# slimgroup/dfno

Hardware: NVIDIA H100
Metric: 3D Navier-Stokes FNO training step (fwd+loss+bwd+Adam) samples/sec, whole job, device-timed, max over ranks (higher is better)
Workload: dtype bf16; 1 GPU; model=FNO3d+t 128^3x20t width 20 modes (12, 12, 12, 10) blocks 4, global_batch=1, seq_len=41943040, parallelism=y-pencil 1x1 (model parallel: field over y, spectral weights over kz), step=forward + DistributedRelativeLpLoss + backward + Adam

## Files before the change

### dfno_b200/csrc/head_sm90.cu

```cuda
#include <type_traits>

#include "head_common.cuh"
#include "kernels.h"
#include "tma_host.h"

namespace dfno {
namespace {

constexpr int kStagesHF = 6;
constexpr int kGroupsHF = 2;
static_assert(kStagesHF % kGroupsHF == 0, "every ring stage must belong to one consumer warpgroup");
constexpr int kThreadsHF = 128 * kGroupsHF + 32;

struct HeadFwdParams {
  int B, C, KR;
  long long S, tiles_per_b;
  const float* w4b4;
  float* out;
  RowMap map;
};


template <int KR, bool kPad>
__device__ __forceinline__ void head_fwd_body(const CUtensorMap& tmH, const CUtensorMap& tmW3, const HeadFwdParams p,
                                              const PadRowMap pm) {
  extern __shared__ __align__(1024) uint8_t smem[];
  constexpr uint32_t w3_bytes = KR > 64 ? 32768u : 16384u;
  uint8_t* s_w3 = smem;
  uint8_t* s_a = smem + w3_bytes;
  constexpr uint32_t half_bytes = KR * 128;
  constexpr uint32_t stage_bytes = 2 * half_bytes;
  uint64_t* bars = reinterpret_cast<uint64_t*>(s_a + kStagesHF * stage_bytes);
  uint64_t* full = bars;
  uint64_t* empty = bars + 6;
  uint64_t* wfull = bars + 12;
  uint32_t* s_w4 = reinterpret_cast<uint32_t*>(bars + 14);
  float* s_b4 = reinterpret_cast<float*>(s_w4 + 64);

  const int warp = __shfl_sync(0xffffffffu, static_cast<int>(threadIdx.x >> 5), 0), lane = threadIdx.x & 31;
  const long long num_tiles = p.tiles_per_b * p.B;

  for (uint32_t i = threadIdx.x; i < kStagesHF * stage_bytes / 16; i += blockDim.x)
    reinterpret_cast<uint4*>(s_a)[i] = make_uint4(0, 0, 0, 0);
  __syncthreads();
  for (uint32_t i = threadIdx.x; i < kStagesHF * 2 * 16; i += blockDim.x) {
    const uint32_t hb = i >> 4, ch = i & 15;
    reinterpret_cast<uint2*>(s_a + hb * half_bytes + p.C * 128)[ch] = make_uint2(0x3F803F80u, 0x3F803F80u);
  }
  for (int i = threadIdx.x; i < 64; i += blockDim.x)
    s_w4[i] = h2_bits(h2_from_f32(p.w4b4[2 * i], p.w4b4[2 * i + 1]));
  if (threadIdx.x == 0) s_b4[0] = p.w4b4[kHidH];
  if (threadIdx.x == 0) {
    tma_prefetch_desc(&tmH); tma_prefetch_desc(&tmW3);
    for (int s = 0; s < kStagesHF; ++s) { mbar_init(&full[s], 1); mbar_init(&empty[s], 1); }
    mbar_init(wfull, 1);
    fence_barrier_init();
  }
  fence_proxy_async_smem();
  __syncthreads();

  if (warp == 4 * kGroupsHF) {
    if (lane == 0) {
      mbar_arrive_expect_tx(wfull, w3_bytes);
      tma_load_2d(s_w3, &tmW3, wfull, 0, 0);
      if constexpr (KR > 64) tma_load_2d(s_w3 + 16384, &tmW3, wfull, 64, 0);
      uint32_t s = 0, ph = 0;
      for (long long tile = blockIdx.x; tile < num_tiles; tile += gridDim.x) {
        const int b = static_cast<int>(tile / p.tiles_per_b);
        const int p0 = static_cast<int>((tile % p.tiles_per_b) * 128);
        mbar_wait(&empty[s], ph ^ 1);
        mbar_arrive_expect_tx(&full[s], 2u * p.C * 128);
        uint8_t* st = s_a + s * stage_bytes;
        tma_load_2d(st, &tmH, &full[s], p0, b * p.C);
        tma_load_2d(st + half_bytes, &tmH, &full[s], p0 + 64, b * p.C);
        if (++s == kStagesHF) { s = 0; ph ^= 1; }
      }
    }
    return;
  }
  const int q = warp & 3, g = warp >> 2, cq = lane & 3;
  const int my_row = frag_row(q, lane, cq);
  const float b4 = s_b4[0];
  const uint32_t w_addr = smem_u32(s_w3);
  uint32_t w4[16];
#pragma unroll
  for (int j = 0; j < 16; ++j) w4[j] = s_w4[4 * j + cq];
  mbar_wait(wfull, 0);
  float acc[128];
  long long n = 0;
  for (long long tile = blockIdx.x; tile < num_tiles; tile += gridDim.x, ++n) {
    if (n % kGroupsHF != g) continue;
    const uint32_t s = static_cast<uint32_t>(n % kStagesHF);
    const int b = static_cast<int>(tile / p.tiles_per_b);
    const long long pos = (tile % p.tiles_per_b) * 128 + my_row;
    mbar_wait(&full[s], (n / kStagesHF) & 1);
    const uint32_t abase = smem_u32(s_a + s * stage_bytes);
    wgmma_fence();
#pragma unroll
    for (int ks = 0; ks < KR / 16; ++ks) {
      const uint32_t w_k = KR > 64 ? (ks >> 2) * 16384 + (ks & 3) * 32 : ks * 32;
      wg_mma128<false, 1, 0>(acc, kHidH, gdesc_mn128(abase + ks * 2048, half_bytes, 1024), half_bytes,
                             gdesc_k128(w_addr + w_k), ks > 0 ? 1u : 0u);
    }
    wgmma_commit();
    wgmma_wait<0>();
    acc_fence(acc);
    if (q == 0 && lane == 0) mbar_arrive(&empty[s]);
    float out[4];
#pragma unroll
    for (int k = 0; k < 4; ++k) {
      const float* a = acc + 64 * (k >> 1) + 2 * (k & 1);
      float sum = 0.f;
#pragma unroll
      for (int half = 0; half < 2; ++half) {
        __half2 part = __float2half2_rn(0.f);
#pragma unroll
        for (int j = 8 * half; j < 8 * half + 8; ++j)
          part = __hfma2(gelu_h2(h2_from_f32(a[4 * j], a[4 * j + 1])), h2_of_bits(w4[j]), part);
        const float2 f = __half22float2(part);
        sum += f.x + f.y;
      }
      sum += __shfl_xor_sync(0xffffffffu, sum, 1);
      sum += __shfl_xor_sync(0xffffffffu, sum, 2);
      out[k] = sum;
    }
    if constexpr (kPad) {
      const long long o = pos < p.S ? pad_row_to_offset(pm, static_cast<uint32_t>(b * p.S + pos)) : -1;
      if (o >= 0) p.out[o] = b4 + pick4(out, cq);
    } else {
      if (pos < p.S) p.out[row_to_offset(p.map, static_cast<uint32_t>(b * p.S + pos))] = b4 + pick4(out, cq);
    }
  }
}

template <int KR>
__global__ void __launch_bounds__(kThreadsHF, 1)
head_fwd_kernel(const __grid_constant__ CUtensorMap tmH, const __grid_constant__ CUtensorMap tmW3,
                const HeadFwdParams p) {
  head_fwd_body<KR, false>(tmH, tmW3, p, PadRowMap{});
}

template <int KR>
__global__ void __launch_bounds__(kThreadsHF, 1)
head_fwd_pad_kernel(const __grid_constant__ CUtensorMap tmH, const __grid_constant__ CUtensorMap tmW3,
                    const HeadFwdParams p, const __grid_constant__ PadRowMap pm) {
  head_fwd_body<KR, true>(tmH, tmW3, p, pm);
}

constexpr int kMaxStagesHB = 6;
constexpr int kGroupsHB = 2;
constexpr int kThreadsHB = 128 * kGroupsHB + 128;
constexpr int kProducerRegsHB = 24, kConsumerRegsHB = 240;
static_assert(128 * kProducerRegsHB + 128 * kGroupsHB * kConsumerRegsHB <= 65536, "register file");
template <int KR>
constexpr bool kWideHB = KR > 48;
template <int KR>
constexpr bool kWsumSmem = KR > 32 && !kWideHB<KR>;
template <int KR>
constexpr int kWsumSmemW = !kWideHB<KR> ? 0 : KR > 64 ? 24 : 32;

struct HeadBwdParams {
  int B, C, KR, stages;
  long long S, tiles_per_b;
  const float* dout;
  const float* amax;
  const float* W4;
  float* gW3; float* gb3; float* gW4; float* gb4;
  RowMap map;
};

template <int KR, bool kPad>
__device__ __forceinline__ void head_bwd2_body(const CUtensorMap& tmH, const CUtensorMap& tmW3, const CUtensorMap& tmW3T,
                                               const CUtensorMap& tmG, const HeadBwdParams p, const PadRowMap pm) {
  extern __shared__ __align__(1024) uint8_t smem[];
  constexpr uint32_t half_bytes = KR * 128;
  constexpr uint32_t tile_bytes = 2 * half_bytes;
  constexpr uint32_t w3_bytes = KR > 64 ? 32768u : 16384u;
  uint8_t* s_w3 = smem;
  uint8_t* s_w3t = s_w3 + w3_bytes;
  uint8_t* s_p = s_w3t + tile_bytes;
  uint8_t* s_a = s_p + kGroupsHB * 32768;
  uint8_t* s_hs = s_a + p.stages * tile_bytes;
  uint8_t* s_g = kWideHB<KR> ? s_hs : s_hs + kGroupsHB * tile_bytes;
  float* s_wsum = reinterpret_cast<float*>(s_g + kGroupsHB * tile_bytes);
  uint64_t* bars = reinterpret_cast<uint64_t*>(s_wsum + (kWsumSmem<KR> ? 32 * 128 * kGroupsHB : 0) +
                                               kWsumSmemW<KR> * 128 * kGroupsHB);
  uint64_t* a_full = bars;
  uint64_t* a_empty = bars + 8;
  uint64_t* w_full = bars + 16;
  float* s_gb4 = reinterpret_cast<float*>(bars + 18);
  uint32_t* s_w4h = reinterpret_cast<uint32_t*>(bars + 20);
  float* s_gw4 = reinterpret_cast<float*>(s_w4h + 64);

  const int warp = __shfl_sync(0xffffffffu, static_cast<int>(threadIdx.x >> 5), 0), lane = threadIdx.x & 31;
  const long long num_tiles = p.tiles_per_b * p.B;

  for (uint32_t i = threadIdx.x; i < p.stages * tile_bytes / 16; i += blockDim.x)
    reinterpret_cast<uint4*>(s_a)[i] = make_uint4(0, 0, 0, 0);
  for (uint32_t i = threadIdx.x; i < kGroupsHB * tile_bytes / 16; i += blockDim.x)
    reinterpret_cast<uint4*>(s_hs)[i] = make_uint4(0, 0, 0, 0);
  __syncthreads();
  for (uint32_t i = threadIdx.x; i < static_cast<uint32_t>(p.stages) * 2 * 16; i += blockDim.x) {
    const uint32_t hb = i >> 4, ch = i & 15;
    reinterpret_cast<uint2*>(s_a + hb * half_bytes + p.C * 128)[ch] = make_uint2(0x3F803F80u, 0x3F803F80u);
  }
  if (threadIdx.x == 0) s_gb4[0] = 0.f;
  for (int i = threadIdx.x; i < 64; i += blockDim.x) s_w4h[i] = h2_bits(h2_from_f32(p.W4[2 * i], p.W4[2 * i + 1]));
  for (int i = threadIdx.x; i < kHidH; i += blockDim.x) s_gw4[i] = 0.f;
  if (threadIdx.x == 0) {
    tma_prefetch_desc(&tmH); tma_prefetch_desc(&tmW3); tma_prefetch_desc(&tmW3T); tma_prefetch_desc(&tmG);
    for (int s = 0; s < p.stages; ++s) { mbar_init(&a_full[s], 1); mbar_init(&a_empty[s], 1); }
    mbar_init(w_full, 1);
    fence_barrier_init();
  }
  fence_proxy_async_smem();
  __syncthreads();
  const float amax = *p.amax;
  const float scale = amax > 0.f ? exp2f(-ceilf(log2f(amax))) : 1.0f;

  if (warp >= 4 * kGroupsHB) {
    setmaxnreg_dec<kProducerRegsHB>();
    if (warp == 4 * kGroupsHB && lane == 0) {
      mbar_arrive_expect_tx(w_full, w3_bytes + tile_bytes);
      tma_load_2d(s_w3, &tmW3, w_full, 0, 0);
      if constexpr (KR > 64) tma_load_2d(s_w3 + 16384, &tmW3, w_full, 64, 0);
      tma_load_2d(s_w3t, &tmW3T, w_full, 0, 0);
      tma_load_2d(s_w3t + half_bytes, &tmW3T, w_full, 64, 0);
      uint32_t s = 0, ph = 0;
      for (long long tile = blockIdx.x; tile < num_tiles; tile += gridDim.x) {
        const int b = static_cast<int>(tile / p.tiles_per_b);
        const int p0 = static_cast<int>((tile % p.tiles_per_b) * 128);
        mbar_wait(&a_empty[s], ph ^ 1);
        mbar_arrive_expect_tx(&a_full[s], 2u * p.C * 128);
        uint8_t* st = s_a + s * tile_bytes;
        tma_load_2d(st, &tmH, &a_full[s], p0, b * p.C);
        tma_load_2d(st + half_bytes, &tmH, &a_full[s], p0 + 64, b * p.C);
        if (++s == static_cast<uint32_t>(p.stages)) { s = 0; ph ^= 1; }
      }
    }
    return;
  }

  setmaxnreg_inc<kConsumerRegsHB>();
  const int q = warp & 3, g = warp >> 2, cq = lane & 3;
  const int my_row = frag_row(q, lane, cq);
  const uint32_t barid = 1 + g;
  const bool leader = q == 0 && lane == 0;
  uint8_t* pbuf = s_p + g * 32768;
  uint8_t* hsbuf = s_hs + g * tile_bytes;
  uint8_t* gbuf = s_g + g * tile_bytes;
  const uint32_t w3_addr = smem_u32(s_w3), w3t_addr = smem_u32(s_w3t);
  const uint32_t p_addr = smem_u32(pbuf), hs_addr = smem_u32(hsbuf), g_addr = smem_u32(gbuf);
  const int mi = lane >> 3, mk = lane & 7;
  const uint32_t p_row = 16 * q + 8 * (mi & 1) + mk;
  const uint32_t g_chunk = 2 * q + (mi & 1);
  float acc_gb4 = 0.f;
  float wsum[32];
  float* my_wsum = s_wsum + (threadIdx.x & (128 * kGroupsHB - 1));
#pragma unroll
  for (int i = 0; i < 32; ++i) {
    if constexpr (kWsumSmem<KR>) my_wsum[i * 128 * kGroupsHB] = 0.f;
    else if constexpr (kWideHB<KR>) { if (i < kWsumSmemW<KR>) my_wsum[i * 128 * kGroupsHB] = 0.f; else wsum[i] = 0.f; }
    else wsum[i] = 0.f;
  }
  auto wsum_add = [&](int i, float d, float v) {
    if constexpr (kWsumSmem<KR>) my_wsum[i * 128 * kGroupsHB] = fmaf(d, v, my_wsum[i * 128 * kGroupsHB]);
    else if constexpr (kWideHB<KR>) {
      if (i < kWsumSmemW<KR>) my_wsum[i * 128 * kGroupsHB] = fmaf(d, v, my_wsum[i * 128 * kGroupsHB]);
      else wsum[i] = fmaf(d, v, wsum[i]);
    } else wsum[i] = fmaf(d, v, wsum[i]);
  };
  float d3[KR];
  uint32_t pa[2][4][4];
  auto mma2 = [&](float (&acc2)[KR], int kb) {
    if constexpr (!kWideHB<KR>) {
#pragma unroll
      for (int ks = 0; ks < 4; ++ks) {
        const uint64_t db = gdesc_k128(w3t_addr + kb * half_bytes + ks * 32);
        const uint32_t sc = (kb > 0 || ks > 0) ? 1u : 0u;
        wg_mma64_rs<KR, 0, 0>(acc2, pa[0][ks], db, sc);
        wg_mma64_rs<KR, 0, KR / 2>(acc2, pa[1][ks], db, sc);
      }
    }
  };
  auto mma2_group = [&](auto c0_, auto ng_, const float (&dk)[4]) {
    constexpr int c0 = decltype(c0_)::value, NG = decltype(ng_)::value;
    float a2[NG];
    wgmma_fence();
#pragma unroll
    for (int ks = 0; ks < 8; ++ks) {
      const uint32_t kb = ks >> 2, kk = ks & 3;
      wg_mma128<true, 0, 0>(a2, NG, gdesc_k128(p_addr + kb * 16384 + kk * 32), 8192,
                            gdesc_k128(w3t_addr + kb * half_bytes + c0 * 128 + kk * 32), ks > 0 ? 1u : 0u);
    }
    wgmma_commit();
    wgmma_wait<0>();
    acc_fence(a2);
#pragma unroll
    for (int mh = 0; mh < 2; ++mh) {
#pragma unroll
      for (int t = 0; t < NG / 16; ++t) {
        uint32_t r[4];
#pragma unroll
        for (int i = 0; i < 4; ++i) {
          const float* a = a2 + (NG / 2) * mh + 4 * (2 * t + (i >> 1)) + 2 * (i & 1);
          const float d = dk[2 * mh + (i & 1)];
          r[i] = pack_bf16x2(d * a[0], d * a[1]);
        }
        const uint32_t c = c0 + 16 * t + 8 * (mi >> 1) + mk;
        stmatrix_x4_trans(g_addr + mh * half_bytes + c * 128 + ((g_chunk ^ (c & 7)) << 4), r);
      }
    }
  };
  long long n = 0, mine = 0;
  mbar_wait(w_full, 0);
  for (long long tile = blockIdx.x; tile < num_tiles; tile += gridDim.x, ++n) {
    if (n % kGroupsHB != g) continue;
    const uint32_t s = static_cast<uint32_t>(n % p.stages);
    const int b = static_cast<int>(tile / p.tiles_per_b);
    const long long p0 = (tile % p.tiles_per_b) * 128;
    const long long pos = p0 + my_row;
    float dl;
    if constexpr (kPad) {
      const long long o = pos < p.S ? pad_row_to_offset(pm, static_cast<uint32_t>(b * p.S + pos)) : -1;
      dl = o >= 0 ? p.dout[o] : 0.f;
    } else {
      dl = pos < p.S ? p.dout[row_to_offset(p.map, static_cast<uint32_t>(b * p.S + pos))] : 0.f;
    }
    acc_gb4 += dl;
    float dk[4];
#pragma unroll
    for (int k = 0; k < 4; ++k) dk[k] = __shfl_sync(0xffffffffu, dl, (lane & ~3) | k);
    mbar_wait(&a_full[s], (n / p.stages) & 1);
    const uint32_t abase = smem_u32(s_a + s * tile_bytes);
    float acc2[KR];
    if constexpr (kWideHB<KR>) {
#pragma unroll
      for (int hq = 0; hq < 4; ++hq) {
        float acc[32];
        wgmma_fence();
#pragma unroll
        for (int ks = 0; ks < KR / 16; ++ks) {
          const uint32_t w_k = KR > 64 ? (ks >> 2) * 16384 + (ks & 3) * 32 : ks * 32;
          wg_mma128<false, 1, 0>(acc, 32, gdesc_mn128(abase + ks * 2048, half_bytes, 1024), half_bytes,
                                 gdesc_k128(w3_addr + hq * 4096 + w_k), ks > 0 ? 1u : 0u);
        }
        wgmma_commit();
        wgmma_wait<0>();
        acc_fence(acc);
        const int hh = hq >> 1;
#pragma unroll
        for (int mh = 0; mh < 2; ++mh) {
#pragma unroll
          for (int kq = 0; kq < 2; ++kq) {
            const int ks = 2 * (hq & 1) + kq;
            uint32_t pr[4];
            afrag_from_acc(acc + 16 * mh, kq, pr, [&](float lo, float hi, int i) {
              const int j = 2 * ks + (i >> 1);
              const GeluH2 vg = gelu_vg_h2(h2_from_f32(lo, hi));
              const float2 a = __half22float2(vg.value);
              const float d = dk[2 * mh + (i & 1)];
              wsum_add(16 * hh + 2 * j, d, a.x);
              wsum_add(16 * hh + 2 * j + 1, d, a.y);
              return h2_bits(__hmul2(vg.grad, h2_of_bits(s_w4h[32 * hh + 4 * j + cq])));
            });
            const uint32_t row = 64 * mh + p_row, chunk = 2 * ks + (mi >> 1);
            stmatrix_x4(p_addr + hh * 16384 + row * 128 + ((chunk ^ (row & 7)) << 4), pr);
          }
        }
      }
    } else {
#pragma unroll
      for (int hh = 0; hh < 2; ++hh) {
        float acc[64];
        wgmma_fence();
#pragma unroll
        for (int ks = 0; ks < KR / 16; ++ks)
          wg_mma128<false, 1, 0>(acc, 64, gdesc_mn128(abase + ks * 2048, half_bytes, 1024), half_bytes,
                                 gdesc_k128(w3_addr + hh * 8192 + ks * 32), ks > 0 ? 1u : 0u);
        wgmma_commit();
        wgmma_wait<0>();
        acc_fence(acc);
#pragma unroll
        for (int mh = 0; mh < 2; ++mh) {
#pragma unroll
          for (int ks = 0; ks < 4; ++ks) {
            afrag_from_acc(acc + 32 * mh, ks, pa[mh][ks], [&](float lo, float hi, int i) {
              const int j = 2 * ks + (i >> 1);
              const GeluH2 vg = gelu_vg_h2(h2_from_f32(lo, hi));
              const float2 a = __half22float2(vg.value);
              const float d = dk[2 * mh + (i & 1)];
              wsum_add(16 * hh + 2 * j, d, a.x);
              wsum_add(16 * hh + 2 * j + 1, d, a.y);
              return h2_bits(__hmul2(vg.grad, h2_of_bits(s_w4h[32 * hh + 4 * j + cq])));
            });
            const uint32_t row = 64 * mh + p_row, chunk = 2 * ks + (mi >> 1);
            stmatrix_x4(p_addr + hh * 16384 + row * 128 + ((chunk ^ (row & 7)) << 4), pa[mh][ks]);
          }
        }
        if (hh == 0) {
          wgmma_fence();
          mma2(acc2, 0);
          wgmma_commit();
          wgmma_wait<0>();
        }
      }
    }
    if constexpr (kWideHB<KR>) {
      if (leader) tma_store_wait_read();
      asm volatile("bar.sync %0, 128;" ::"r"(barid) : "memory");
      const uint8_t* src = s_a + s * tile_bytes;
#pragma unroll 1
      for (int k = 0; k < 4; ++k) {
        const int row = frag_row(q, lane, k);
        const float ds = dk[k] * scale;
        const uint32_t colo = (row >> 6) * half_bytes + ((row & 7) << 1);
        const uint32_t ch = (row & 63) >> 3;
#pragma unroll
        for (int cc = 0; cc < KR / 4; ++cc) {
          const int c = 4 * cc + cq;
          const uint32_t off = colo + c * 128 + ((ch ^ (c & 7)) << 4);
          if (c < p.C) {
            const uint16_t hv = *reinterpret_cast<const uint16_t*>(src + off);
            *reinterpret_cast<__half*>(hsbuf + off) = __float2half_rn(__uint_as_float(static_cast<uint32_t>(hv) << 16) * ds);
          } else if (c == p.C) {
            *reinterpret_cast<__half*>(hsbuf + off) = __float2half_rn(ds);
          }
        }
      }

      fence_proxy_async_smem();
      asm volatile("bar.sync %0, 128;" ::"r"(barid) : "memory");
      if (leader) mbar_arrive(&a_empty[s]);
      wgmma_fence();
#pragma unroll
      for (int ks = 0; ks < 8; ++ks) {
        const uint32_t kb = ks >> 2, kk = ks & 3;
        wg_mma128<true, 1, 0>(d3, KR, gdesc_mn128(p_addr + ks * 2048, 16384, 1024), 16384,
                              gdesc_k128(hs_addr + kb * half_bytes + kk * 32), (mine > 0 || ks > 0) ? 1u : 0u);
      }
      wgmma_commit();
      wgmma_wait<0>();
      acc_fence(d3);
      ++mine;
      constexpr int kG0 = KR > 64 ? 48 : 32;
      mma2_group(std::integral_constant<int, 0>{}, std::integral_constant<int, kG0>{}, dk);
      mma2_group(std::integral_constant<int, kG0>{}, std::integral_constant<int, KR - kG0>{}, dk);
      fence_proxy_async_smem();
      asm volatile("bar.sync %0, 128;" ::"r"(barid) : "memory");
      if (leader) {
        const int row0 = b * p.C;
        tma_store_2d(&tmG, gbuf, static_cast<int32_t>(p0), row0);
        if (p0 + 64 < p.S) tma_store_2d(&tmG, gbuf + half_bytes, static_cast<int32_t>(p0 + 64), row0);
        tma_store_commit();
      }
      continue;
    }
    {
      const uint8_t* src = s_a + s * tile_bytes;
#pragma unroll
      for (int k = 0; k < 4; ++k) {
        const int row = frag_row(q, lane, k);
        const float ds = dk[k] * scale;
        const uint32_t colo = (row >> 6) * half_bytes + ((row & 7) << 1);
        const uint32_t ch = (row & 63) >> 3;
#pragma unroll
        for (int cc = 0; cc < KR / 4; ++cc) {
          const int c = 4 * cc + cq;
          const uint32_t off = colo + c * 128 + ((ch ^ (c & 7)) << 4);
          if (c < p.C) {
            const uint16_t hv = *reinterpret_cast<const uint16_t*>(src + off);
            *reinterpret_cast<__half*>(hsbuf + off) = __float2half_rn(__uint_as_float(static_cast<uint32_t>(hv) << 16) * ds);
          } else if (c == p.C) {
            *reinterpret_cast<__half*>(hsbuf + off) = __float2half_rn(ds);
          }
        }
    }
    }
    if (leader) tma_store_wait_read();
    fence_proxy_async_smem();
    asm volatile("bar.sync %0, 128;" ::"r"(barid) : "memory");
    wgmma_fence();
    mma2(acc2, 1);
#pragma unroll
    for (int ks = 0; ks < 8; ++ks) {
      const uint32_t kb = ks >> 2, kk = ks & 3;
      wg_mma128<true, 1, 0>(d3, KR, gdesc_mn128(p_addr + ks * 2048, 16384, 1024), 16384,
                            gdesc_k128(hs_addr + kb * half_bytes + kk * 32), (mine > 0 || ks > 0) ? 1u : 0u);
    }
    wgmma_commit();
    wgmma_wait<0>();
    acc_fence(acc2);
    acc_fence(d3);
    ++mine;
    if (leader) mbar_arrive(&a_empty[s]);
#pragma unroll
    for (int mh = 0; mh < 2; ++mh) {
#pragma unroll
      for (int t = 0; t < KR / 16; ++t) {
        uint32_t r[4];
#pragma unroll
        for (int i = 0; i < 4; ++i) {
          const float* a = acc2 + (KR / 2) * mh + 4 * (2 * t + (i >> 1)) + 2 * (i & 1);
          const float d = dk[2 * mh + (i & 1)];
          r[i] = pack_bf16x2(d * a[0], d * a[1]);
        }
        const uint32_t c = 16 * t + 8 * (mi >> 1) + mk;
        stmatrix_x4_trans(g_addr + mh * half_bytes + c * 128 + ((g_chunk ^ (c & 7)) << 4), r);
      }
    }
    fence_proxy_async_smem();
    asm volatile("bar.sync %0, 128;" ::"r"(barid) : "memory");
    if (leader) {
      const int row0 = b * p.C;
      tma_store_2d(&tmG, gbuf, static_cast<int32_t>(p0), row0);
      if (p0 + 64 < p.S) tma_store_2d(&tmG, gbuf + half_bytes, static_cast<int32_t>(p0 + 64), row0);
      tma_store_commit();
    }
  }
  if (leader) tma_store_wait_all();
  acc_gb4 += __shfl_xor_sync(0xffffffffu, acc_gb4, 16);
  acc_gb4 += __shfl_xor_sync(0xffffffffu, acc_gb4, 8);
  acc_gb4 += __shfl_xor_sync(0xffffffffu, acc_gb4, 4);
  acc_gb4 += __shfl_xor_sync(0xffffffffu, acc_gb4, 2);
  acc_gb4 += __shfl_xor_sync(0xffffffffu, acc_gb4, 1);
  if (lane == 0) atomicAdd(s_gb4, acc_gb4);
#pragma unroll
  for (int i = 0; i < 32; ++i) {
    float v = kWsumSmem<KR> || i < kWsumSmemW<KR> ? my_wsum[i * 128 * kGroupsHB] : wsum[i];
    v += __shfl_xor_sync(0xffffffffu, v, 4);
    v += __shfl_xor_sync(0xffffffffu, v, 8);
    v += __shfl_xor_sync(0xffffffffu, v, 16);
    if (lane < 4) atomicAdd(&s_gw4[64 * (i >> 4) + 8 * ((i & 15) >> 1) + 2 * cq + (i & 1)], v);
  }
  if (mine > 0) {
    const float inv = 1.0f / scale;
#pragma unroll
    for (int h = 0; h < 2; ++h)
#pragma unroll
      for (int j = 0; j < KR / 8; ++j)
#pragma unroll
        for (int e = 0; e < 4; ++e) {
          const int hid = 64 * h + 16 * q + (lane >> 2) + 8 * (e >> 1), c = 8 * j + 2 * (lane & 3) + (e & 1);
          const float v = d3[(KR / 2) * h + 4 * j + e] * inv;
          {
            if (c < p.C) atomicAdd(p.gW3 + hid * p.C + c, v);
            else if (c == p.C) atomicAdd(p.gb3 + hid, v);
          }
        }
  }
  asm volatile("bar.sync 3, %0;" ::"n"(128 * kGroupsHB) : "memory");
  if (num_tiles > blockIdx.x && threadIdx.x < kHidH) {
    atomicAdd(p.gW4 + threadIdx.x, s_gw4[threadIdx.x]);
    if (threadIdx.x == 0) atomicAdd(p.gb4, s_gb4[0]);
  }
}

template <int KR>
__global__ void __launch_bounds__(kThreadsHB, 1)
head_bwd2_kernel(const __grid_constant__ CUtensorMap tmH, const __grid_constant__ CUtensorMap tmW3,
                 const __grid_constant__ CUtensorMap tmW3T, const __grid_constant__ CUtensorMap tmG,
                 const HeadBwdParams p) {
  head_bwd2_body<KR, false>(tmH, tmW3, tmW3T, tmG, p, PadRowMap{});
}

template <int KR>
__global__ void __launch_bounds__(kThreadsHB, 1)
head_bwd2_pad_kernel(const __grid_constant__ CUtensorMap tmH, const __grid_constant__ CUtensorMap tmW3,
                     const __grid_constant__ CUtensorMap tmW3T, const __grid_constant__ CUtensorMap tmG,
                     const HeadBwdParams p, const __grid_constant__ PadRowMap pm) {
  head_bwd2_body<KR, true>(tmH, tmW3, tmW3T, tmG, p, pm);
}

}

const char* head_fwd(const void* h, const void* W3aug, const float* w4b4, float* out, int B, int C, long long S,
                     int nrl, const int* R, const long long* SR, const int* lim, int num_sms, cudaStream_t stream) {
  if (C < 1 || C > 64) return "head_fwd: 1 <= C <= 64";
  if (S % 8 || S > (1ll << 31) - 256 || static_cast<long long>(B) * S > (1ll << 31) - 256) return "head_fwd: bad slab size";
  HeadFwdParams p{};
  p.B = B; p.C = C; p.KR = (C + 1 + 15) / 16 * 16; p.S = S; p.tiles_per_b = (S + 127) / 128;
  p.w4b4 = w4b4; p.out = out;
  PadRowMap pm{};
  if (lim ? set_padrowmap(&pm, nrl, R, SR, lim) : set_rowmap(&p.map, nrl, R, SR))
    return lim ? "head_fwd: 1..5 row digits, each bound within its radix" : "head_fwd: 1..4 row digits";
  CUtensorMap tmH, tmW3;
  if (make_map_2d(&tmH, h, S, static_cast<uint64_t>(B) * C, S, 64, C)) return "tensor map (h) failed";
  const int w3_cols = p.KR > 64 ? 128 : 64;
  if (make_map_2d(&tmW3, W3aug, w3_cols, 128, w3_cols, 64, 128)) return "tensor map (W3) failed";
  static bool attr[2][5] = {};
  const int kr_i = p.KR / 16 - 1, pd = lim ? 1 : 0;
  const void* fns[2][5] = {{reinterpret_cast<const void*>(head_fwd_kernel<16>),
                            reinterpret_cast<const void*>(head_fwd_kernel<32>),
                            reinterpret_cast<const void*>(head_fwd_kernel<48>),
                            reinterpret_cast<const void*>(head_fwd_kernel<64>),
                            reinterpret_cast<const void*>(head_fwd_kernel<80>)},
                           {reinterpret_cast<const void*>(head_fwd_pad_kernel<16>),
                            reinterpret_cast<const void*>(head_fwd_pad_kernel<32>),
                            reinterpret_cast<const void*>(head_fwd_pad_kernel<48>),
                            reinterpret_cast<const void*>(head_fwd_pad_kernel<64>),
                            reinterpret_cast<const void*>(head_fwd_pad_kernel<80>)}};
  const void* fn = fns[pd][kr_i];
  if (!attr[pd][kr_i]) {
    if (cudaFuncSetAttribute(fn, cudaFuncAttributeMaxDynamicSharedMemorySize, 227 * 1024) != cudaSuccess)
      return "cudaFuncSetAttribute failed";
    attr[pd][kr_i] = true;
  }
  const uint32_t smem_bytes = (p.KR > 64 ? 32768 : 16384) + kStagesHF * 2 * p.KR * 128 + 2048 + 1024;
  const long long tiles = p.tiles_per_b * B;
  const int grid = static_cast<int>(tiles < num_sms ? tiles : num_sms);
#define DFNO_HEAD_FWD(K_, ...)                                                                         \
  if (kr_i == 0) K_<16><<<grid, kThreadsHF, smem_bytes, stream>>>(__VA_ARGS__);                          \
  else if (kr_i == 1) K_<32><<<grid, kThreadsHF, smem_bytes, stream>>>(__VA_ARGS__);                     \
  else if (kr_i == 2) K_<48><<<grid, kThreadsHF, smem_bytes, stream>>>(__VA_ARGS__);                     \
  else if (kr_i == 3) K_<64><<<grid, kThreadsHF, smem_bytes, stream>>>(__VA_ARGS__);                     \
  else K_<80><<<grid, kThreadsHF, smem_bytes, stream>>>(__VA_ARGS__);
  if (pd) { DFNO_HEAD_FWD(head_fwd_pad_kernel, tmH, tmW3, p, pm) } else { DFNO_HEAD_FWD(head_fwd_kernel, tmH, tmW3, p) }
#undef DFNO_HEAD_FWD
  cudaError_t e = cudaGetLastError();
  return e == cudaSuccess ? nullptr : cudaGetErrorString(e);
}

const char* head_bwd2(const void* h, const void* W3aug, const void* W3T16, const float* W4, const float* dout,
                      long long n_dout, unsigned* amax_ws, void* g, float* gW3, float* gb3, float* gW4, float* gb4,
                      int B, int C, long long S, int nrl, const int* R, const long long* SR, const int* lim,
                      int num_sms, cudaStream_t stream) {
  if (C < 1 || C > 64) return "head_bwd: 1 <= C <= 64";
  if (S % 8 || S > (1ll << 31) - 256 || static_cast<long long>(B) * S > (1ll << 31) - 256) return "head_bwd: bad slab size";
  HeadBwdParams p{};
  p.B = B; p.C = C; p.KR = (C + 1 + 15) / 16 * 16; p.S = S; p.tiles_per_b = (S + 127) / 128;
  p.dout = dout; p.amax = reinterpret_cast<const float*>(amax_ws); p.W4 = W4;
  p.gW3 = gW3; p.gb3 = gb3; p.gW4 = gW4; p.gb4 = gb4;
  PadRowMap pm{};
  if (lim ? set_padrowmap(&pm, nrl, R, SR, lim) : set_rowmap(&p.map, nrl, R, SR))
    return lim ? "head_bwd: 1..5 row digits, each bound within its radix" : "head_bwd: 1..4 row digits";
  CUtensorMap tmH, tmW3, tmW3T, tmG;
  if (make_map_2d(&tmH, h, S, static_cast<uint64_t>(B) * C, S, 64, C)) return "tensor map (h) failed";
  const int w3_cols = p.KR > 64 ? 128 : 64;
  if (make_map_2d(&tmW3, W3aug, w3_cols, 128, w3_cols, 64, 128)) return "tensor map (W3) failed";
  if (make_map_2d(&tmW3T, W3T16, 128, p.KR, 128, 64, p.KR)) return "tensor map (W3T) failed";
  if (make_map_2d(&tmG, g, S, static_cast<uint64_t>(B) * C, S, 64, C)) return "tensor map (g) failed";
  static bool attr[2][5] = {};
  const int kr_i = p.KR / 16 - 1, pd = lim ? 1 : 0;
  const void* fns[2][5] = {{reinterpret_cast<const void*>(head_bwd2_kernel<16>),
                            reinterpret_cast<const void*>(head_bwd2_kernel<32>),
                            reinterpret_cast<const void*>(head_bwd2_kernel<48>),
                            reinterpret_cast<const void*>(head_bwd2_kernel<64>),
                            reinterpret_cast<const void*>(head_bwd2_kernel<80>)},
                           {reinterpret_cast<const void*>(head_bwd2_pad_kernel<16>),
                            reinterpret_cast<const void*>(head_bwd2_pad_kernel<32>),
                            reinterpret_cast<const void*>(head_bwd2_pad_kernel<48>),
                            reinterpret_cast<const void*>(head_bwd2_pad_kernel<64>),
                            reinterpret_cast<const void*>(head_bwd2_pad_kernel<80>)}};
  const void* fn = fns[pd][kr_i];
  if (!attr[pd][kr_i]) {
    if (cudaFuncSetAttribute(fn, cudaFuncAttributeMaxDynamicSharedMemorySize, 227 * 1024) != cudaSuccess)
      return "cudaFuncSetAttribute failed";
    attr[pd][kr_i] = true;
  }
  if (cudaMemsetAsync(amax_ws, 0, 4, stream) != cudaSuccess) return "head_bwd: memset failed";
  absmax_kernel<<<num_sms * 4, 256, 0, stream>>>(dout, n_dout, amax_ws);
  const uint32_t tile_bytes = 2u * p.KR * 128;
  const bool wide = p.KR > 48;
  const uint32_t wsum_n = !wide ? (p.KR > 32 ? 32 : 0) : p.KR > 64 ? 24 : 32;
  const uint32_t fixed = (p.KR > 64 ? 32768 : 16384) + tile_bytes + kGroupsHB * (32768 + (wide ? 1 : 2) * tile_bytes) +
                         2048 + 1024 + wsum_n * 128 * kGroupsHB * 4;
  p.stages = kMaxStagesHB;
  while (p.stages > kGroupsHB && fixed + p.stages * tile_bytes > 227 * 1024) p.stages -= kGroupsHB;
  if (fixed + p.stages * tile_bytes > 227 * 1024) return "head_bwd: tile does not fit shared memory";
  const uint32_t smem_bytes = fixed + p.stages * tile_bytes;
  const long long tiles = p.tiles_per_b * B;
  const int grid = static_cast<int>(tiles < num_sms ? tiles : num_sms);
#define DFNO_HEAD_BWD(K_, ...)                                                                         \
  if (kr_i == 0) K_<16><<<grid, kThreadsHB, smem_bytes, stream>>>(__VA_ARGS__);                          \
  else if (kr_i == 1) K_<32><<<grid, kThreadsHB, smem_bytes, stream>>>(__VA_ARGS__);                     \
  else if (kr_i == 2) K_<48><<<grid, kThreadsHB, smem_bytes, stream>>>(__VA_ARGS__);                     \
  else if (kr_i == 3) K_<64><<<grid, kThreadsHB, smem_bytes, stream>>>(__VA_ARGS__);                     \
  else K_<80><<<grid, kThreadsHB, smem_bytes, stream>>>(__VA_ARGS__);
  if (pd) { DFNO_HEAD_BWD(head_bwd2_pad_kernel, tmH, tmW3, tmW3T, tmG, p, pm) }
  else { DFNO_HEAD_BWD(head_bwd2_kernel, tmH, tmW3, tmW3T, tmG, p) }
#undef DFNO_HEAD_BWD
  cudaError_t e = cudaGetLastError();
  return e == cudaSuccess ? nullptr : cudaGetErrorString(e);
}

}
```

Before: 16.56 samples/s.

## Software-pipeline head forward and backward wgmma with epilogues for narrow KR

For KR<=48 the head forward kernel splits each tile's first GEMM into two 64-column halves and interleaves two tiles per iteration. Async wgmma for one half then overlaps the GELU/dot epilogue of the other, and the stage is released early. For non-wide KR the backward kernel is restructured the same way: a register-fed mma2 becomes an smem-descriptor wgmma issued asynchronously alongside the second-half GEMM, the hs copy is overlapped, dout is prefetched one tile ahead, and the d3 accumulation is waited lazily. This adds code complexity and changes barrier ordering. The hs copy also drops the c>=C guard and the bias column written at c==C, which may be a correctness risk.

```diff
diff --git a/dfno_b200/csrc/head_sm90.cu b/dfno_b200/csrc/head_sm90.cu
--- a/dfno_b200/csrc/head_sm90.cu
+++ b/dfno_b200/csrc/head_sm90.cu
@@ -86,6 +86,82 @@
 #pragma unroll
   for (int j = 0; j < 16; ++j) w4[j] = s_w4[4 * j + cq];
   mbar_wait(wfull, 0);
+  if constexpr (KR <= 48) {
+    float acc0[64], acc1[64];
+    auto mma_half = [&](float (&a)[64], long long m, int hh) {
+      const uint32_t abase = smem_u32(s_a + static_cast<uint32_t>(m % kStagesHF) * stage_bytes);
+      wgmma_fence();
+#pragma unroll
+      for (int ks = 0; ks < KR / 16; ++ks)
+        wg_mma128<false, 1, 0>(a, 64, gdesc_mn128(abase + ks * 2048, half_bytes, 1024), half_bytes,
+                               gdesc_k128(w_addr + hh * 8192 + ks * 32), ks > 0 ? 1u : 0u);
+      wgmma_commit();
+    };
+    auto dot_half = [&](const float (&a)[64], int k, int hh) {
+      const float* r = a + 32 * (k >> 1) + 2 * (k & 1);
+      __half2 part = __float2half2_rn(0.f);
+#pragma unroll
+      for (int j = 0; j < 8; ++j)
+        part = __hfma2(gelu_h2(h2_from_f32(r[4 * j], r[4 * j + 1])), h2_of_bits(w4[8 * hh + j]), part);
+      const float2 f = __half22float2(part);
+      return f.x + f.y;
+    };
+    auto epi0 = [&](float (&sum)[4]) {
+      acc_fence(acc0);
+#pragma unroll
+      for (int k = 0; k < 4; ++k) {
+        sum[k] = 0.f;
+        sum[k] += dot_half(acc0, k, 0);
+      }
+    };
+    auto epi1 = [&](const float (&sum)[4], long long t) {
+      acc_fence(acc1);
+      float out[4];
+#pragma unroll
+      for (int k = 0; k < 4; ++k) {
+        float s = sum[k];
+        s += dot_half(acc1, k, 1);
+        s += __shfl_xor_sync(0xffffffffu, s, 1);
+        s += __shfl_xor_sync(0xffffffffu, s, 2);
+        out[k] = s;
+      }
+      const int b = static_cast<int>(t / p.tiles_per_b);
+      const long long pos = (t % p.tiles_per_b) * 128 + my_row;
+      if constexpr (kPad) {
+        const long long o = pos < p.S ? pad_row_to_offset(pm, static_cast<uint32_t>(b * p.S + pos)) : -1;
+        if (o >= 0) p.out[o] = b4 + pick4(out, cq);
+      } else {
+        if (pos < p.S) p.out[row_to_offset(p.map, static_cast<uint32_t>(b * p.S + pos))] = b4 + pick4(out, cq);
+      }
+    };
+    const long long step = static_cast<long long>(kGroupsHF) * gridDim.x;
+    long long n = g;
+    for (long long tile = blockIdx.x + static_cast<long long>(g) * gridDim.x; tile < num_tiles;
+         tile += 2 * step, n += 2 * kGroupsHF) {
+      const bool two = tile + step < num_tiles;
+      const long long n1 = two ? n + kGroupsHF : n;
+      float sum[4];
+      mbar_wait(&full[n % kStagesHF], (n / kStagesHF) & 1);
+      mma_half(acc0, n, 0);
+      mma_half(acc1, n, 1);
+      wgmma_wait<1>();
+      epi0(sum);
+      if (two) mbar_wait(&full[n1 % kStagesHF], (n1 / kStagesHF) & 1);
+      mma_half(acc0, n1, 0);
+      wgmma_wait<1>();
+      if (q == 0 && lane == 0) mbar_arrive(&empty[n % kStagesHF]);
+      epi1(sum, tile);
+      mma_half(acc1, n1, 1);
+      wgmma_wait<1>();
+      epi0(sum);
+      wgmma_wait<0>();
+      if (two) {
+        if (q == 0 && lane == 0) mbar_arrive(&empty[n1 % kStagesHF]);
+        epi1(sum, tile + step);
+      }
+    }
+    return;
+  }
   float acc[128];
   long long n = 0;
   for (long long tile = blockIdx.x; tile < num_tiles; tile += gridDim.x, ++n) {
@@ -271,18 +347,6 @@
     } else wsum[i] = fmaf(d, v, wsum[i]);
   };
   float d3[KR];
-  uint32_t pa[2][4][4];
-  auto mma2 = [&](float (&acc2)[KR], int kb) {
-    if constexpr (!kWideHB<KR>) {
-#pragma unroll
-      for (int ks = 0; ks < 4; ++ks) {
-        const uint64_t db = gdesc_k128(w3t_addr + kb * half_bytes + ks * 32);
-        const uint32_t sc = (kb > 0 || ks > 0) ? 1u : 0u;
-        wg_mma64_rs<KR, 0, 0>(acc2, pa[0][ks], db, sc);
-        wg_mma64_rs<KR, 0, KR / 2>(acc2, pa[1][ks], db, sc);
-      }
-    }
-  };
   auto mma2_group = [&](auto c0_, auto ng_, const float (&dk)[4]) {
     constexpr int c0 = decltype(c0_)::value, NG = decltype(ng_)::value;
     float a2[NG];
@@ -314,27 +378,164 @@
   };
   long long n = 0, mine = 0;
   mbar_wait(w_full, 0);
-  for (long long tile = blockIdx.x; tile < num_tiles; tile += gridDim.x, ++n) {
-    if (n % kGroupsHB != g) continue;
-    const uint32_t s = static_cast<uint32_t>(n % p.stages);
-    const int b = static_cast<int>(tile / p.tiles_per_b);
-    const long long p0 = (tile % p.tiles_per_b) * 128;
-    const long long pos = p0 + my_row;
-    float dl;
-    if constexpr (kPad) {
-      const long long o = pos < p.S ? pad_row_to_offset(pm, static_cast<uint32_t>(b * p.S + pos)) : -1;
-      dl = o >= 0 ? p.dout[o] : 0.f;
-    } else {
-      dl = pos < p.S ? p.dout[row_to_offset(p.map, static_cast<uint32_t>(b * p.S + pos))] : 0.f;
-    }
-    acc_gb4 += dl;
-    float dk[4];
-#pragma unroll
-    for (int k = 0; k < 4; ++k) dk[k] = __shfl_sync(0xffffffffu, dl, (lane & ~3) | k);
-    mbar_wait(&a_full[s], (n / p.stages) & 1);
-    const uint32_t abase = smem_u32(s_a + s * tile_bytes);
-    float acc2[KR];
-    if constexpr (kWideHB<KR>) {
+  if constexpr (!kWideHB<KR>) {
+    auto load_dout = [&](long long t) {
+      const int b = static_cast<int>(t / p.tiles_per_b);
+      const long long pos = (t % p.tiles_per_b) * 128 + my_row;
+      if constexpr (kPad) {
+        const long long o = pos < p.S ? pad_row_to_offset(pm, static_cast<uint32_t>(b * p.S + pos)) : -1;
+        return o >= 0 ? p.dout[o] : 0.f;
+      } else {
+        return pos < p.S ? p.dout[row_to_offset(p.map, static_cast<uint32_t>(b * p.S + pos))] : 0.f;
+      }
+    };
+    auto mma1 = [&](float (&acc)[64], uint32_t abase, int hh) {
+      wgmma_fence();
+#pragma unroll
+      for (int ks = 0; ks < KR / 16; ++ks)
+        wg_mma128<false, 1, 0>(acc, 64, gdesc_mn128(abase + ks * 2048, half_bytes, 1024), half_bytes,
+                               gdesc_k128(w3_addr + hh * 8192 + ks * 32), ks > 0 ? 1u : 0u);
+      wgmma_commit();
+    };
+    auto mma2 = [&](float (&acc2)[KR], int kb) {
+      wgmma_fence();
+#pragma unroll
+      for (int ks = 0; ks < 4; ++ks)
+        wg_mma128<true, 0, 0>(acc2, KR, gdesc_k128(p_addr + kb * 16384 + ks * 32), 8192,
+                              gdesc_k128(w3t_addr + kb * half_bytes + ks * 32), (kb > 0 || ks > 0) ? 1u : 0u);
+      wgmma_commit();
+    };
+    auto epi_a = [&](const float (&acc)[64], int hh, const float (&dk)[4]) {
+#pragma unroll
+      for (int mh = 0; mh < 2; ++mh) {
+#pragma unroll
+        for (int ks = 0; ks < 4; ++ks) {
+          uint32_t pr[4];
+          afrag_from_acc(acc + 32 * mh, ks, pr, [&](float lo, float hi, int i) {
+            const int j = 2 * ks + (i >> 1);
+            const GeluH2 vg = gelu_vg_h2(h2_from_f32(lo, hi));
+            const float2 a = __half22float2(vg.value);
+            const float d = dk[2 * mh + (i & 1)];
+            wsum_add(16 * hh + 2 * j, d, a.x);
+            wsum_add(16 * hh + 2 * j + 1, d, a.y);
+            return h2_bits(__hmul2(vg.grad, h2_of_bits(s_w4h[32 * hh + 4 * j + cq])));
+          });
+          const uint32_t row = 64 * mh + p_row, chunk = 2 * ks + (mi >> 1);
+          stmatrix_x4(p_addr + hh * 16384 + row * 128 + ((chunk ^ (row & 7)) << 4), pr);
+        }
+      }
+    };
+    auto hs_copy = [&](uint32_t s, const float (&dk)[4]) {
+      const uint8_t* src = s_a + s * tile_bytes;
+#pragma unroll
+      for (int k = 0; k < 4; ++k) {
+        const int row = frag_row(q, lane, k);
+        const float ds = dk[k] * scale;
+        const uint32_t colo = (row >> 6) * half_bytes + ((row & 7) << 1);
+        const uint32_t ch = (row & 63) >> 3;
+#pragma unroll
+        for (int cc = 0; cc < KR / 4; ++cc) {
+          const int c = 4 * cc + cq;
+          const uint32_t off = colo + c * 128 + ((ch ^ (c & 7)) << 4);
+          const uint16_t hv = *reinterpret_cast<const uint16_t*>(src + off);
+          *reinterpret_cast<__half*>(hsbuf + off) = __float2half_rn(__uint_as_float(static_cast<uint32_t>(hv) << 16) * ds);
+        }
+      }
+    };
+    const long long step = static_cast<long long>(kGroupsHB) * gridDim.x;
+    long long tile = blockIdx.x + static_cast<long long>(g) * gridDim.x;
+    n = g;
+    float dl_next = tile < num_tiles ? load_dout(tile) : 0.f;
+    for (; tile < num_tiles; tile += step, n += kGroupsHB) {
+      const uint32_t s = static_cast<uint32_t>(n % p.stages);
+      const int b = static_cast<int>(tile / p.tiles_per_b);
+      const long long p0 = (tile % p.tiles_per_b) * 128;
+      const float dl = dl_next;
+      if (tile + step < num_tiles) dl_next = load_dout(tile + step);
+      acc_gb4 += dl;
+      float dk[4];
+#pragma unroll
+      for (int k = 0; k < 4; ++k) dk[k] = __shfl_sync(0xffffffffu, dl, (lane & ~3) | k);
+      mbar_wait(&a_full[s], (n / p.stages) & 1);
+      const uint32_t abase = smem_u32(s_a + s * tile_bytes);
+      float acc2[KR];
+      float acc[64];
+      mma1(acc, abase, 0);
+      wgmma_wait<0>();
+      acc_fence(acc);
+      acc_fence(d3);
+      epi_a(acc, 0, dk);
+      fence_proxy_async_smem();
+      asm volatile("bar.sync %0, 128;" ::"r"(barid) : "memory");
+      mma2(acc2, 0);
+      mma1(acc, abase, 1);
+      if constexpr (KR <= 32) hs_copy(s, dk);
+      wgmma_wait<0>();
+      acc_fence(acc);
+      epi_a(acc, 1, dk);
+      if constexpr (KR > 32) hs_copy(s, dk);
+      if (leader) tma_store_wait_read();
+      fence_proxy_async_smem();
+      asm volatile("bar.sync %0, 128;" ::"r"(barid) : "memory");
+      if (leader) mbar_arrive(&a_empty[s]);
+      mma2(acc2, 1);
+      wgmma_fence();
+#pragma unroll
+      for (int ks = 0; ks < 8; ++ks) {
+        const uint32_t kb = ks >> 2, kk = ks & 3;
+        wg_mma128<true, 1, 0>(d3, KR, gdesc_mn128(p_addr + ks * 2048, 16384, 1024), 16384,
+                              gdesc_k128(hs_addr + kb * half_bytes + kk * 32), (mine > 0 || ks > 0) ? 1u : 0u);
+      }
+      wgmma_commit();
+      ++mine;
+      wgmma_wait<1>();
+      acc_fence(acc2);
+#pragma unroll
+      for (int mh = 0; mh < 2; ++mh) {
+#pragma unroll
+        for (int t = 0; t < KR / 16; ++t) {
+          uint32_t r[4];
+#pragma unroll
+          for (int i = 0; i < 4; ++i) {
+            const float* a = acc2 + (KR / 2) * mh + 4 * (2 * t + (i >> 1)) + 2 * (i & 1);
+            const float d = dk[2 * mh + (i & 1)];
+            r[i] = pack_bf16x2(d * a[0], d * a[1]);
+          }
+          const uint32_t c = 16 * t + 8 * (mi >> 1) + mk;
+          stmatrix_x4_trans(g_addr + mh * half_bytes + c * 128 + ((g_chunk ^ (c & 7)) << 4), r);
+        }
+      }
+      fence_proxy_async_smem();
+      asm volatile("bar.sync %0, 128;" ::"r"(barid) : "memory");
+      if (leader) {
+        const int row0 = b * p.C;
+        tma_store_2d(&tmG, gbuf, static_cast<int32_t>(p0), row0);
+        if (p0 + 64 < p.S) tma_store_2d(&tmG, gbuf + half_bytes, static_cast<int32_t>(p0 + 64), row0);
+        tma_store_commit();
+      }
+    }
+    wgmma_wait<0>();
+    acc_fence(d3);
+  } else {
+    for (long long tile = blockIdx.x; tile < num_tiles; tile += gridDim.x, ++n) {
+      if (n % kGroupsHB != g) continue;
+      const uint32_t s = static_cast<uint32_t>(n % p.stages);
+      const int b = static_cast<int>(tile / p.tiles_per_b);
+      const long long p0 = (tile % p.tiles_per_b) * 128;
+      const long long pos = p0 + my_row;
+      float dl;
+      if constexpr (kPad) {
+        const long long o = pos < p.S ? pad_row_to_offset(pm, static_cast<uint32_t>(b * p.S + pos)) : -1;
+        dl = o >= 0 ? p.dout[o] : 0.f;
+      } else {
+        dl = pos < p.S ? p.dout[row_to_offset(p.map, static_cast<uint32_t>(b * p.S + pos))] : 0.f;
+      }
+      acc_gb4 += dl;
+      float dk[4];
+#pragma unroll
+      for (int k = 0; k < 4; ++k) dk[k] = __shfl_sync(0xffffffffu, dl, (lane & ~3) | k);
+      mbar_wait(&a_full[s], (n / p.stages) & 1);
+      const uint32_t abase = smem_u32(s_a + s * tile_bytes);
 #pragma unroll
       for (int hq = 0; hq < 4; ++hq) {
         float acc[32];
@@ -369,44 +570,6 @@
           }
         }
       }
-    } else {
-#pragma unroll
-      for (int hh = 0; hh < 2; ++hh) {
-        float acc[64];
-        wgmma_fence();
-#pragma unroll
-        for (int ks = 0; ks < KR / 16; ++ks)
-          wg_mma128<false, 1, 0>(acc, 64, gdesc_mn128(abase + ks * 2048, half_bytes, 1024), half_bytes,
-                                 gdesc_k128(w3_addr + hh * 8192 + ks * 32), ks > 0 ? 1u : 0u);
-        wgmma_commit();
-        wgmma_wait<0>();
-        acc_fence(acc);
-#pragma unroll
-        for (int mh = 0; mh < 2; ++mh) {
-#pragma unroll
-          for (int ks = 0; ks < 4; ++ks) {
-            afrag_from_acc(acc + 32 * mh, ks, pa[mh][ks], [&](float lo, float hi, int i) {
-              const int j = 2 * ks + (i >> 1);
-              const GeluH2 vg = gelu_vg_h2(h2_from_f32(lo, hi));
-              const float2 a = __half22float2(vg.value);
-              const float d = dk[2 * mh + (i & 1)];
-              wsum_add(16 * hh + 2 * j, d, a.x);
-              wsum_add(16 * hh + 2 * j + 1, d, a.y);
-              return h2_bits(__hmul2(vg.grad, h2_of_bits(s_w4h[32 * hh + 4 * j + cq])));
-            });
-            const uint32_t row = 64 * mh + p_row, chunk = 2 * ks + (mi >> 1);
-            stmatrix_x4(p_addr + hh * 16384 + row * 128 + ((chunk ^ (row & 7)) << 4), pa[mh][ks]);
-          }
-        }
-        if (hh == 0) {
-          wgmma_fence();
-          mma2(acc2, 0);
-          wgmma_commit();
-          wgmma_wait<0>();
-        }
-      }
-    }
-    if constexpr (kWideHB<KR>) {
       if (leader) tma_store_wait_read();
       asm volatile("bar.sync %0, 128;" ::"r"(barid) : "memory");
       const uint8_t* src = s_a + s * tile_bytes;
@@ -428,7 +591,6 @@
           }
         }
       }
-
       fence_proxy_async_smem();
       asm volatile("bar.sync %0, 128;" ::"r"(barid) : "memory");
       if (leader) mbar_arrive(&a_empty[s]);
@@ -454,68 +616,6 @@
         if (p0 + 64 < p.S) tma_store_2d(&tmG, gbuf + half_bytes, static_cast<int32_t>(p0 + 64), row0);
         tma_store_commit();
       }
-      continue;
-    }
-    {
-      const uint8_t* src = s_a + s * tile_bytes;
-#pragma unroll
-      for (int k = 0; k < 4; ++k) {
-        const int row = frag_row(q, lane, k);
-        const float ds = dk[k] * scale;
-        const uint32_t colo = (row >> 6) * half_bytes + ((row & 7) << 1);
-        const uint32_t ch = (row & 63) >> 3;
-#pragma unroll
-        for (int cc = 0; cc < KR / 4; ++cc) {
-          const int c = 4 * cc + cq;
-          const uint32_t off = colo + c * 128 + ((ch ^ (c & 7)) << 4);
-          if (c < p.C) {
-            const uint16_t hv = *reinterpret_cast<const uint16_t*>(src + off);
-            *reinterpret_cast<__half*>(hsbuf + off) = __float2half_rn(__uint_as_float(static_cast<uint32_t>(hv) << 16) * ds);
-          } else if (c == p.C) {
-            *reinterpret_cast<__half*>(hsbuf + off) = __float2half_rn(ds);
-          }
-        }
-    }
-    }
-    if (leader) tma_store_wait_read();
-    fence_proxy_async_smem();
-    asm volatile("bar.sync %0, 128;" ::"r"(barid) : "memory");
-    wgmma_fence();
-    mma2(acc2, 1);
-#pragma unroll
-    for (int ks = 0; ks < 8; ++ks) {
-      const uint32_t kb = ks >> 2, kk = ks & 3;
-      wg_mma128<true, 1, 0>(d3, KR, gdesc_mn128(p_addr + ks * 2048, 16384, 1024), 16384,
-                            gdesc_k128(hs_addr + kb * half_bytes + kk * 32), (mine > 0 || ks > 0) ? 1u : 0u);
-    }
-    wgmma_commit();
-    wgmma_wait<0>();
-    acc_fence(acc2);
-    acc_fence(d3);
-    ++mine;
-    if (leader) mbar_arrive(&a_empty[s]);
-#pragma unroll
-    for (int mh = 0; mh < 2; ++mh) {
-#pragma unroll
-      for (int t = 0; t < KR / 16; ++t) {
-        uint32_t r[4];
-#pragma unroll
-        for (int i = 0; i < 4; ++i) {
-          const float* a = acc2 + (KR / 2) * mh + 4 * (2 * t + (i >> 1)) + 2 * (i & 1);
-          const float d = dk[2 * mh + (i & 1)];
-          r[i] = pack_bf16x2(d * a[0], d * a[1]);
-        }
-        const uint32_t c = 16 * t + 8 * (mi >> 1) + mk;
-        stmatrix_x4_trans(g_addr + mh * half_bytes + c * 128 + ((g_chunk ^ (c & 7)) << 4), r);
-      }
-    }
-    fence_proxy_async_smem();
-    asm volatile("bar.sync %0, 128;" ::"r"(barid) : "memory");
-    if (leader) {
-      const int row0 = b * p.C;
-      tma_store_2d(&tmG, gbuf, static_cast<int32_t>(p0), row0);
-      if (p0 + 64 < p.S) tma_store_2d(&tmG, gbuf + half_bytes, static_cast<int32_t>(p0 + 64), row0);
-      tma_store_commit();
     }
   }
   if (leader) tma_store_wait_all();
```

Result: faster. 16.98 samples/s, median of 6 (+2.5%).
